# dongyunjinyu/YOLO-Lite

Hardware: NVIDIA B200
Metric: images_per_sec (higher is better)
Workload: dtype bf16

## Files before the change

### yolo-lite_b200/csrc/c3k2_fused.cu

```cuda
#include "common.cuh"

namespace yl {

struct C3k2TailParams {
    const __nv_bfloat16* t;
    long long t_cstride;
    int t_coff;
    __nv_bfloat16* y;
    long long y_cstride;
    int y_coff;
    const __nv_bfloat16 *wa, *wb, *w2;
    const float *ba, *bb, *b2;
    int wa_rows, wa_k, wb_k, w2_k;
    int N, H, W, C2, add;
    int tiles_w, tiles_h, total_tiles;
};

__device__ __forceinline__ void ldsm_x4(uint32_t addr, uint32_t& r0, uint32_t& r1, uint32_t& r2, uint32_t& r3) {
    asm volatile("ldmatrix.sync.aligned.m8n8.x4.shared.b16 {%0,%1,%2,%3}, [%4];"
                 : "=r"(r0), "=r"(r1), "=r"(r2), "=r"(r3)
                 : "r"(addr));
}
__device__ __forceinline__ void ldsm_x2(uint32_t addr, uint32_t& r0, uint32_t& r1) {
    asm volatile("ldmatrix.sync.aligned.m8n8.x2.shared.b16 {%0,%1}, [%2];" : "=r"(r0), "=r"(r1) : "r"(addr));
}
__device__ __forceinline__ void mma16816(float (&d)[4], const uint32_t (&a)[4], uint32_t b0, uint32_t b1) {
    asm volatile(
        "mma.sync.aligned.m16n8k16.row.col.f32.bf16.bf16.f32 {%0,%1,%2,%3}, {%4,%5,%6,%7}, {%8,%9}, {%0,%1,%2,%3};"
        : "+f"(d[0]), "+f"(d[1]), "+f"(d[2]), "+f"(d[3])
        : "r"(a[0]), "r"(a[1]), "r"(a[2]), "r"(a[3]), "r"(b0), "r"(b1));
}

__host__ __device__ constexpr int pitch16(int data_bytes) { return data_bytes + (((data_bytes / 16) & 1) ? 32 : 16); }

template <int C>
struct C3k2Smem {
    static constexpr int CH = C / 2;
    static constexpr int TH = (C == 16) ? 16 : 8, TW = 16;
    static constexpr int PH = TH + 4, PW = TW + 4;
    static constexpr int HH = TH + 2, HW = TW + 2;
    static constexpr int TS = pitch16(4 * C);
    static constexpr int HS = pitch16(2 * CH);
    static constexpr int YS = pitch16(2 * C);
    static constexpr int KA = 9 * C, KB = 9 * CH, K2 = 3 * C;
    static constexpr int WAS = pitch16(2 * KA), WBS = pitch16(2 * KB + 16), W2S = pitch16(2 * K2);
    static constexpr int NA = CH < 16 ? 8 : CH;
    static constexpr int HM = (HH * HW + 15) / 16;
    static constexpr int NBUF = C == 16 ? 2 : 1;
    static constexpr int T_BYTES = PH * PW * TS;
    static constexpr int off_t = 0;
    static constexpr int off_h = off_t + NBUF * T_BYTES;
    static constexpr int off_y2 = off_h + HM * 16 * HS;
    static constexpr int off_wa = off_y2 + TH * TW * YS;
    static constexpr int off_wb = off_wa + NA * WAS;
    static constexpr int off_w2 = off_wb + C * WBS;
    __host__ __device__ static constexpr int w2_bytes(int c2) { return c2 * W2S; }
    __host__ __device__ static constexpr int bias_floats(int c2) { return NA + C + c2; }
    __host__ __device__ static constexpr int total(int c2) { return off_w2 + w2_bytes(c2) + bias_floats(c2) * 4; }
};

__device__ __forceinline__ void stage_weights(uint8_t* dst, const __nv_bfloat16* src, int rows, int src_rows, int kbytes,
                                              int pitch) {
    const int units = pitch / 16;
    for (int i = threadIdx.x; i < rows * units; i += blockDim.x) {
        const int r = i / units, u = i - r * units;
        uint4 v = make_uint4(0u, 0u, 0u, 0u);
        if (r < src_rows && u * 16 < kbytes)
            v = __ldg(reinterpret_cast<const uint4*>(reinterpret_cast<const uint8_t*>(src) + (size_t)r * kbytes) + u);
        *reinterpret_cast<uint4*>(dst + (size_t)r * pitch + u * 16) = v;
    }
}

template <int C>
__global__ void __launch_bounds__(256, 2) c3k2_tail_kernel(const C3k2TailParams p) {
    using S = C3k2Smem<C>;
    constexpr int CH = S::CH, TH = S::TH, TW = S::TW, PW = S::PW, HW = S::HW, HH = S::HH;
    constexpr int TS = S::TS, HS = S::HS, YS = S::YS, WAS = S::WAS, WBS = S::WBS, W2S = S::W2S;
    extern __shared__ __align__(16) uint8_t smem[];
    griddep_launch_dependents();
    const int lane = threadIdx.x & 31, warp = threadIdx.x >> 5;
    const int g = lane >> 2, t = lane & 3;
    const int lrow = lane & 15, khalf = lane >> 4;
    const uint32_t sT = smem_u32(smem + S::off_t), sH = smem_u32(smem + S::off_h), sY2 = smem_u32(smem + S::off_y2);
    const uint32_t sWa = smem_u32(smem + S::off_wa), sWb = smem_u32(smem + S::off_wb), sW2 = smem_u32(smem + S::off_w2);
    float* sba = reinterpret_cast<float*>(smem + S::off_w2 + S::w2_bytes(p.C2));
    float* sbb = sba + S::NA;
    float* sb2 = sbb + C;

    stage_weights(smem + S::off_wa, p.wa, S::NA, p.wa_rows, p.wa_k * 2, WAS);
    stage_weights(smem + S::off_wb, p.wb, C, C, p.wb_k * 2, WBS);
    stage_weights(smem + S::off_w2, p.w2, p.C2, p.C2, p.w2_k * 2, W2S);
    for (int i = threadIdx.x; i < S::NA; i += blockDim.x) sba[i] = i < CH ? __ldg(p.ba + i) : 0.f;
    for (int i = threadIdx.x; i < C; i += blockDim.x) sbb[i] = __ldg(p.bb + i);
    for (int i = threadIdx.x; i < p.C2; i += blockDim.x) sb2[i] = __ldg(p.b2 + i);
    __syncthreads();

    constexpr int KT = 2 * C / 16, KY = C / 16, KC = KT + KY;
    const int NG = p.C2 / 32;
    const int grp = warp % NG, rblk = warp / NG;
    uint32_t bC[KC][4][2];
#pragma unroll
    for (int ks = 0; ks < KC; ++ks)
#pragma unroll
        for (int np = 0; np < 2; ++np)
            ldsm_x4(sW2 + (uint32_t)((grp * 32 + np * 16 + (lane >> 4) * 8 + (lane & 7)) * W2S + (ks * 16 + 8 * ((lane >> 3) & 1)) * 2),
                    bC[ks][2 * np][0], bC[ks][2 * np][1], bC[ks][2 * np + 1][0], bC[ks][2 * np + 1][1]);
    constexpr bool THIN = (C == 16);
    constexpr int KSB = (9 * CH + 15) / 16;
    uint32_t bA[THIN ? 9 : 1][2];
    if (THIN) {
#pragma unroll
        for (int tap = 0; tap < 9; ++tap)
            ldsm_x2(sWa + (uint32_t)((lane & 7) * WAS + (tap * C + 8 * ((lane >> 3) & 1)) * 2), bA[THIN ? tap : 0][0],
                    bA[THIN ? tap : 0][1]);
    }
    griddep_wait();

    constexpr int CHUNKS = 4 * C / 16;
    auto load_patch = [&](int tile, uint32_t dst) {
        const int w0 = (tile % p.tiles_w) * TW;
        const int h0 = ((tile / p.tiles_w) % p.tiles_h) * TH;
        const int n = tile / (p.tiles_w * p.tiles_h);
        const __nv_bfloat16* src0 = p.t + (long long)n * p.H * p.W * p.t_cstride + p.t_coff;
        for (int idx = threadIdx.x; idx < S::PH * PW * CHUNKS; idx += blockDim.x) {
            const int pix = idx / CHUNKS, ck = idx - pix * CHUNKS;
            const int pr = pix / PW, pc = pix - pr * PW;
            const int hi = h0 - 2 + pr, wi = w0 - 2 + pc;
            const bool ok = hi >= 0 && hi < p.H && wi >= 0 && wi < p.W;
            const int off = ok ? hi * p.W + wi : 0;
            asm volatile("cp.async.cg.shared.global [%0], [%1], 16, %2;" ::"r"(dst + (uint32_t)(pix * TS + ck * 16)),
                         "l"(src0 + (long long)off * p.t_cstride + ck * 8), "r"(ok ? 16 : 0)
                         : "memory");
        }
        asm volatile("cp.async.commit_group;" ::: "memory");
    };

    int buf = 0;
    if (S::NBUF == 2 && (int)blockIdx.x < p.total_tiles) load_patch(blockIdx.x, sT);
    for (int tile = blockIdx.x; tile < p.total_tiles; tile += gridDim.x) {
        const int w0 = (tile % p.tiles_w) * TW;
        const int h0 = ((tile / p.tiles_w) % p.tiles_h) * TH;
        const int n = tile / (p.tiles_w * p.tiles_h);
        const uint32_t sTc = sT + (uint32_t)(buf * S::T_BYTES);
        if (S::NBUF == 1) load_patch(tile, sTc);
        asm volatile("cp.async.wait_group 0;" ::: "memory");
        __syncthreads();
        if (S::NBUF == 2) {
            if (tile + (int)gridDim.x < p.total_tiles) load_patch(tile + gridDim.x, sT + (uint32_t)((buf ^ 1) * S::T_BYTES));
            buf ^= 1;
        }

        {
            constexpr int NT = (CH + 7) / 8;
            constexpr int KS_TAP = C / 16;
            for (int mt = warp; mt < S::HM; mt += 8) {
                int idx = mt * 16 + lrow;
                idx = idx < HH * HW ? idx : HH * HW - 1;
                const int hr = idx / HW, hc = idx - hr * HW;
                const uint32_t arow = sTc + (uint32_t)((hr * PW + hc) * TS + (C + 8 * khalf) * 2);
                float acc[NT][4];
#pragma unroll
                for (int nt = 0; nt < NT; ++nt) {
                    const float2 bb2 = *reinterpret_cast<const float2*>(sba + nt * 8 + 2 * t);
                    acc[nt][0] = bb2.x; acc[nt][1] = bb2.y; acc[nt][2] = bb2.x; acc[nt][3] = bb2.y;
                }
                if (THIN) {
                    uint32_t a9[9][4];
#pragma unroll
                    for (int tap = 0; tap < 9; ++tap)
                        ldsm_x4(arow + (uint32_t)(((tap / 3) * PW + tap % 3) * TS), a9[tap][0], a9[tap][1], a9[tap][2], a9[tap][3]);
#pragma unroll
                    for (int tap = 0; tap < 9; ++tap) mma16816(acc[0], a9[tap], bA[THIN ? tap : 0][0], bA[THIN ? tap : 0][1]);
                } else {
#pragma unroll
                    for (int tap = 0; tap < 9; ++tap) {
                        const int dr = tap / 3, dc = tap - 3 * dr;
                        uint32_t a[KS_TAP][4], b[KS_TAP][4];
#pragma unroll
                        for (int ks = 0; ks < KS_TAP; ++ks) {
                            ldsm_x4(arow + (uint32_t)((dr * PW + dc) * TS + ks * 32), a[ks][0], a[ks][1], a[ks][2], a[ks][3]);
                            ldsm_x4(sWa + (uint32_t)((((lane >> 4) * 8) + (lane & 7)) * WAS + (tap * C + ks * 16 + 8 * ((lane >> 3) & 1)) * 2),
                                    b[ks][0], b[ks][1], b[ks][2], b[ks][3]);
                        }
#pragma unroll
                        for (int ks = 0; ks < KS_TAP; ++ks) {
                            mma16816(acc[0], a[ks], b[ks][0], b[ks][1]);
                            mma16816(acc[NT - 1], a[ks], b[ks][2], b[ks][3]);
                        }
                    }
                }
#pragma unroll
                for (int half = 0; half < 2; ++half) {
                    const int e = mt * 16 + g + half * 8;
                    if (e >= HH * HW) continue;
                    const int er = e / HW, ec = e - er * HW;
                    const int hi = h0 - 1 + er, wi = w0 - 1 + ec;
                    const bool in = hi >= 0 && hi < p.H && wi >= 0 && wi < p.W;
#pragma unroll
                    for (int nt = 0; nt < NT; ++nt) {
                        const float v0 = in ? silu_fast(acc[nt][half * 2]) : 0.f;
                        const float v1 = in ? silu_fast(acc[nt][half * 2 + 1]) : 0.f;
                        asm volatile("st.shared.b32 [%0], %1;" ::"r"(sH + (uint32_t)(e * HS + (nt * 8 + 2 * t) * 2)),
                                     "r"(pack_bf16x2(v0, v1))
                                     : "memory");
                    }
                }
            }
        }
        __syncthreads();

        for (int r = warp; r < TH; r += 8) {
            constexpr int NT = C / 8;
            float acc[NT][4];
#pragma unroll
            for (int nt = 0; nt < NT; ++nt) {
                const float2 bb2 = *reinterpret_cast<const float2*>(sbb + nt * 8 + 2 * t);
                acc[nt][0] = bb2.x; acc[nt][1] = bb2.y; acc[nt][2] = bb2.x; acc[nt][3] = bb2.y;
            }
            const uint32_t hrow = sH + (uint32_t)((r * HW + lrow) * HS);
            if (CH == 8) {
                uint32_t a[KSB][4], b[KSB][4];
#pragma unroll
                for (int ks = 0; ks < KSB; ++ks) {
                    const int tap = min(2 * ks + khalf, 8);
                    const int dr = tap / 3, dc = tap - 3 * dr;
                    ldsm_x4(hrow + (uint32_t)((dr * HW + dc) * HS), a[ks][0], a[ks][1], a[ks][2], a[ks][3]);
                    ldsm_x4(sWb + (uint32_t)(((lane >> 4) * 8 + (lane & 7)) * WBS + (ks * 16 + 8 * ((lane >> 3) & 1)) * 2),
                            b[ks][0], b[ks][1], b[ks][2], b[ks][3]);
                }
#pragma unroll
                for (int ks = 0; ks < KSB; ++ks) {
                    mma16816(acc[0], a[ks], b[ks][0], b[ks][1]);
                    mma16816(acc[1], a[ks], b[ks][2], b[ks][3]);
                }
            } else {
                constexpr int KS_TAP = CH / 16;
#pragma unroll
                for (int k3 = 0; k3 < KSB; k3 += 3) {
                    uint32_t a[3][4], b[3][NT / 2][4];
#pragma unroll
                    for (int j = 0; j < 3; ++j) {
                        const int ks = k3 + j;
                        const int tap = ks / KS_TAP, kk = ks - tap * KS_TAP;
                        const int dr = tap / 3, dc = tap - 3 * dr;
                        ldsm_x4(hrow + (uint32_t)((dr * HW + dc) * HS + (kk * 16 + 8 * khalf) * 2), a[j][0], a[j][1], a[j][2], a[j][3]);
#pragma unroll
                        for (int np = 0; np < NT / 2; ++np)
                            ldsm_x4(sWb + (uint32_t)((np * 16 + (lane >> 4) * 8 + (lane & 7)) * WBS + (ks * 16 + 8 * ((lane >> 3) & 1)) * 2),
                                    b[j][np][0], b[j][np][1], b[j][np][2], b[j][np][3]);
                    }
#pragma unroll
                    for (int j = 0; j < 3; ++j)
#pragma unroll
                        for (int np = 0; np < NT / 2; ++np) {
                            mma16816(acc[2 * np], a[j], b[j][np][0], b[j][np][1]);
                            mma16816(acc[2 * np + 1], a[j], b[j][np][2], b[j][np][3]);
                        }
                }
            }
#pragma unroll
            for (int half = 0; half < 2; ++half) {
                const int col = g + half * 8;
                const uint32_t y1p = sTc + (uint32_t)(((r + 2) * PW + col + 2) * TS + C * 2);
                const uint32_t y2p = sY2 + (uint32_t)((r * TW + col) * YS);
#pragma unroll
                for (int nt = 0; nt < NT; ++nt) {
                    float v0 = silu_fast(acc[nt][half * 2]), v1 = silu_fast(acc[nt][half * 2 + 1]);
                    if (p.add) {
                        uint32_t rv;
                        asm volatile("ld.shared.b32 %0, [%1];" : "=r"(rv) : "r"(y1p + (uint32_t)((nt * 8 + 2 * t) * 2)));
                        v0 += bf16lo_f(rv);
                        v1 += bf16hi_f(rv);
                    }
                    asm volatile("st.shared.b32 [%0], %1;" ::"r"(y2p + (uint32_t)((nt * 8 + 2 * t) * 2)), "r"(pack_bf16x2(v0, v1))
                                 : "memory");
                }
            }
        }
        __syncthreads();

        {
            const int scol = g + 8 * (t >> 1);
            const int wi = w0 + scol;
            const int rpw = TH * NG / 8;
            for (int rr = 0; rr < rpw; ++rr) {
                const int r = rblk * rpw + rr;
                uint32_t a[KC][4];
                const uint32_t trow = sTc + (uint32_t)(((r + 2) * PW + lrow + 2) * TS + 8 * khalf * 2);
                const uint32_t yrow = sY2 + (uint32_t)((r * TW + lrow) * YS + 8 * khalf * 2);
#pragma unroll
                for (int ks = 0; ks < KT; ++ks) ldsm_x4(trow + ks * 32, a[ks][0], a[ks][1], a[ks][2], a[ks][3]);
#pragma unroll
                for (int ks = 0; ks < KY; ++ks) ldsm_x4(yrow + ks * 32, a[KT + ks][0], a[KT + ks][1], a[KT + ks][2], a[KT + ks][3]);
                float acc[4][4];
#pragma unroll
                for (int nt = 0; nt < 4; ++nt) {
                    const float2 bb2 = *reinterpret_cast<const float2*>(sb2 + grp * 32 + nt * 8 + 2 * t);
                    acc[nt][0] = bb2.x; acc[nt][1] = bb2.y; acc[nt][2] = bb2.x; acc[nt][3] = bb2.y;
                }
#pragma unroll
                for (int ks = 0; ks < KC; ++ks)
#pragma unroll
                    for (int nt = 0; nt < 4; ++nt) mma16816(acc[nt], a[ks], bC[ks][nt][0], bC[ks][nt][1]);
                const int hi = h0 + r;
                const bool st_ok = hi < p.H && wi < p.W;
                __nv_bfloat16* yp = p.y + (((long long)n * p.H + hi) * p.W + wi) * p.y_cstride + p.y_coff + grp * 32 + 8 * (t & 1);
#pragma unroll
                for (int np = 0; np < 2; ++np) {
                    uint32_t v0 = pack_bf16x2(silu_fast(acc[2 * np][0]), silu_fast(acc[2 * np][1]));
                    uint32_t v1 = pack_bf16x2(silu_fast(acc[2 * np + 1][0]), silu_fast(acc[2 * np + 1][1]));
                    uint32_t v2 = pack_bf16x2(silu_fast(acc[2 * np][2]), silu_fast(acc[2 * np][3]));
                    uint32_t v3 = pack_bf16x2(silu_fast(acc[2 * np + 1][2]), silu_fast(acc[2 * np + 1][3]));
                    {
                        const uint32_t s0 = (t & 1) ? v0 : v1, s1 = (t & 1) ? v2 : v3;
                        const uint32_t r0 = __shfl_xor_sync(0xffffffffu, s0, 1), r1 = __shfl_xor_sync(0xffffffffu, s1, 1);
                        if (t & 1) { v0 = r0; v2 = r1; } else { v1 = r0; v3 = r1; }
                    }
                    {
                        const uint32_t s0 = (t & 2) ? v0 : v2, s1 = (t & 2) ? v1 : v3;
                        const uint32_t r0 = __shfl_xor_sync(0xffffffffu, s0, 2), r1 = __shfl_xor_sync(0xffffffffu, s1, 2);
                        if (t & 2) { v0 = r0; v1 = r1; } else { v2 = r0; v3 = r1; }
                    }
                    if (st_ok) *reinterpret_cast<uint4*>(yp + np * 16) = make_uint4(v0, v1, v2, v3);
                }
            }
        }
        __syncthreads();
    }
}

static int g_c3k2_sms = 148, g_c3k2_max_smem = 0;

template <int C>
static int launch_c3k2_tail(C3k2TailParams p, cudaStream_t s) {
    using S = C3k2Smem<C>;
    p.tiles_w = ceil_div(p.W, S::TW);
    p.tiles_h = ceil_div(p.H, S::TH);
    p.total_tiles = p.tiles_w * p.tiles_h * p.N;
    const size_t smem = (size_t)S::total(p.C2);
    YL_CHECK((int)smem <= g_c3k2_max_smem, YL_ERR_UNSUPPORTED, "c3k2 tail needs %zu B of shared memory (device allows %d)", smem,
             g_c3k2_max_smem);
    int per_sm = (int)((size_t)220 * 1024 / (smem + 1024));
    per_sm = per_sm < 1 ? 1 : (per_sm > 2 ? 2 : per_sm);
    int grid = g_c3k2_sms * per_sm;
    if (grid > p.total_tiles) grid = p.total_tiles;
    YL_CUDA(launch_kernel(c3k2_tail_kernel<C>, dim3(grid), dim3(256), smem, s, p));
    YL_LAUNCH_OK("c3k2_tail_kernel");
    return YL_OK;
}

int init_c3k2() {
    int dev = 0;
    YL_CUDA(cudaGetDevice(&dev));
    YL_CUDA(cudaDeviceGetAttribute(&g_c3k2_sms, cudaDevAttrMultiProcessorCount, dev));
    YL_CUDA(cudaDeviceGetAttribute(&g_c3k2_max_smem, cudaDevAttrMaxSharedMemoryPerBlockOptin, dev));
    YL_CUDA(cudaFuncSetAttribute(c3k2_tail_kernel<16>, cudaFuncAttributeMaxDynamicSharedMemorySize, g_c3k2_max_smem));
    YL_CUDA(cudaFuncSetAttribute(c3k2_tail_kernel<32>, cudaFuncAttributeMaxDynamicSharedMemorySize, g_c3k2_max_smem));
    return YL_OK;
}

}

namespace yl {
bool c3k2_tc_supported(int c, int c2);
int launch_c3k2_tc(const yl_tensor* t, const yl_tensor* y, const void* wa, const float* ba, int wa_ci_pad, const void* wb,
                   const float* bb, int wb_ci_pad, const void* w2, const float* b2, int w2_ci_pad, int shortcut,
                   cudaStream_t stream);
}

extern "C" int yl_c3k2_tail_tc(const yl_tensor* t, const yl_tensor* y, const void* wa, const float* ba, int wa_co_pad,
                               int wa_ci_pad, const void* wb, const float* bb, int wb_ci_pad, const void* w2,
                               const float* b2, int w2_ci_pad, int shortcut, void* stream) {
    YL_CHECK(t && y && t->data && y->data && wa && wb && w2 && ba && bb && b2, YL_ERR_ARG, "null pointer");
    YL_CHECK(t->dtype == YL_BF16 && y->dtype == YL_BF16, YL_ERR_ARG, "c3k2 tail tensors must be bf16");
    YL_CHECK(t->n == y->n && t->h == y->h && t->w == y->w && t->c % 32 == 0, YL_ERR_ARG, "c3k2 tail shape mismatch");
    YL_CHECK(t->coff % 8 == 0 && t->cstride % 8 == 0 && y->coff % 8 == 0 && y->cstride % 8 == 0, YL_ERR_ARG,
             "c3k2 tail needs 8-channel alignment");
    const int c = t->c / 2;
    YL_CHECK(wa_co_pad >= c / 2 && wa_ci_pad == c && wb_ci_pad == (c / 2 + 7) / 8 * 8 && w2_ci_pad == 3 * c, YL_ERR_ARG,
             "packed weight layouts do not match the block");
    return yl::launch_c3k2_tc(t, y, wa, ba, wa_ci_pad, wb, bb, wb_ci_pad, w2, b2, w2_ci_pad, shortcut, (cudaStream_t)stream);
}

extern "C" int yl_c3k2_tail_supported(int c, int c2) {
    return (c == 16 || c == 32) && (c2 == 32 || c2 == 64 || c2 == 128 || c2 == 256);
}

extern "C" int yl_c3k2_tail(const yl_tensor* t, const yl_tensor* y, const void* wa, const float* ba, int wa_co_pad,
                            int wa_ci_pad, const void* wb, const float* bb, int wb_ci_pad, const void* w2, const float* b2,
                            int w2_ci_pad, int shortcut, void* stream) {
    YL_CHECK(t && y && t->data && y->data && wa && wb && w2 && ba && bb && b2, YL_ERR_ARG, "null pointer");
    YL_CHECK(t->dtype == YL_BF16 && y->dtype == YL_BF16, YL_ERR_ARG, "c3k2 tail tensors must be bf16");
    YL_CHECK(t->n == y->n && t->h == y->h && t->w == y->w, YL_ERR_ARG, "c3k2 tail shape mismatch");
    YL_CHECK(t->c % 32 == 0 && yl_c3k2_tail_supported(t->c / 2, y->c), YL_ERR_UNSUPPORTED,
             "c3k2 tail is built for c in {16, 32} and c2 in {32, 64, 128, 256} (got c = %d, c2 = %d)", t->c / 2, y->c);
    YL_CHECK(t->coff % 8 == 0 && t->cstride % 8 == 0 && y->coff % 8 == 0 && y->cstride % 8 == 0, YL_ERR_ARG,
             "c3k2 tail needs 8-channel alignment");
    YL_CHECK(((uintptr_t)t->data | (uintptr_t)y->data | (uintptr_t)wa | (uintptr_t)wb | (uintptr_t)w2) % 16 == 0, YL_ERR_ARG,
             "pointers must be 16-byte aligned");
    const int c = t->c / 2;
    YL_CHECK(wa_ci_pad == c && wb_ci_pad == (c / 2 + 7) / 8 * 8 && w2_ci_pad == 3 * c, YL_ERR_ARG,
             "packed weight layouts do not match the block (ci_pad %d / %d / %d for c = %d)", wa_ci_pad, wb_ci_pad,
             w2_ci_pad, c);
    YL_CHECK((long long)t->h * t->w < (1ll << 31), YL_ERR_ARG, "image too large");
    if (yl::c3k2_tc_supported(c, y->c))
        return yl::launch_c3k2_tc(t, y, wa, ba, wa_ci_pad, wb, bb, wb_ci_pad, w2, b2, w2_ci_pad, shortcut, (cudaStream_t)stream);
    yl::C3k2TailParams p;
    p.t = reinterpret_cast<const __nv_bfloat16*>(t->data);
    p.t_cstride = t->cstride;
    p.t_coff = t->coff;
    p.y = reinterpret_cast<__nv_bfloat16*>(y->data);
    p.y_cstride = y->cstride;
    p.y_coff = y->coff;
    p.wa = reinterpret_cast<const __nv_bfloat16*>(wa);
    p.wb = reinterpret_cast<const __nv_bfloat16*>(wb);
    p.w2 = reinterpret_cast<const __nv_bfloat16*>(w2);
    p.ba = ba;
    p.bb = bb;
    p.b2 = b2;
    p.wa_rows = wa_co_pad;
    p.wa_k = 9 * wa_ci_pad;
    p.wb_k = 9 * wb_ci_pad;
    p.w2_k = w2_ci_pad;
    p.N = t->n;
    p.H = t->h;
    p.W = t->w;
    p.C2 = y->c;
    p.add = shortcut;
    cudaStream_t s = (cudaStream_t)stream;
    return c == 16 ? yl::launch_c3k2_tail<16>(p, s) : yl::launch_c3k2_tail<32>(p, s);
}
```

### yolo-lite_b200/csrc/stem_fused.cu

```cuda
#include <cuda_fp16.h>

#include "common.cuh"

namespace yl {

struct StemFusedParams {
    const void* x;
    int N, CI, H, W;
    const __nv_bfloat16* w0;
    int ci_pad0;
    const float* b0;
    const __nv_bfloat16* w1;
    const float* b1;
    __nv_bfloat16* y;
    long long y_cstride;
    int y_coff;
    int H0, W0, H1, W1;
    int act0, act1;
    int tiles_w, tiles_h, total_tiles;
};

__device__ __forceinline__ void sf_ldsm_x4(uint32_t addr, uint32_t& r0, uint32_t& r1, uint32_t& r2, uint32_t& r3) {
    asm volatile("ldmatrix.sync.aligned.m8n8.x4.shared.b16 {%0,%1,%2,%3}, [%4];"
                 : "=r"(r0), "=r"(r1), "=r"(r2), "=r"(r3)
                 : "r"(addr));
}
__device__ __forceinline__ void sf_mma(float (&d)[4], const uint32_t (&a)[4], uint32_t b0, uint32_t b1) {
    asm volatile(
        "mma.sync.aligned.m16n8k16.row.col.f32.bf16.bf16.f32 {%0,%1,%2,%3}, {%4,%5,%6,%7}, {%8,%9}, {%0,%1,%2,%3};"
        : "+f"(d[0]), "+f"(d[1]), "+f"(d[2]), "+f"(d[3])
        : "r"(a[0]), "r"(a[1]), "r"(a[2]), "r"(a[3]), "r"(b0), "r"(b1));
}

template <typename T> struct SfQuad;
template <> struct SfQuad<float> {
    using raw = float4;
    static __device__ __forceinline__ raw zero() { return make_float4(0.f, 0.f, 0.f, 0.f); }
    static __device__ __forceinline__ raw load(const float* p) { return __ldg(reinterpret_cast<const float4*>(p)); }
    static __device__ __forceinline__ float4 widen(raw v) { return v; }
    static __device__ __forceinline__ float one(const float* p) { return __ldg(p); }
};
template <> struct SfQuad<__half> {
    using raw = uint2;
    static __device__ __forceinline__ raw zero() { return make_uint2(0u, 0u); }
    static __device__ __forceinline__ raw load(const __half* p) { return __ldg(reinterpret_cast<const uint2*>(p)); }
    static __device__ __forceinline__ float4 widen(raw v) {
        const float2 a = __half22float2(*reinterpret_cast<const __half2*>(&v.x));
        const float2 b = __half22float2(*reinterpret_cast<const __half2*>(&v.y));
        return make_float4(a.x, a.y, b.x, b.y);
    }
    static __device__ __forceinline__ float one(const __half* p) { return __half2float(*p); }
};
template <> struct SfQuad<uint8_t> {
    using raw = uint32_t;
    static __device__ __forceinline__ raw zero() { return 0u; }
    static __device__ __forceinline__ raw load(const uint8_t* p) { return __ldg(reinterpret_cast<const uint32_t*>(p)); }
    static __device__ __forceinline__ float4 widen(raw v) {
        return make_float4(__fdiv_rn((float)(v & 0xffu), 255.f), __fdiv_rn((float)((v >> 8) & 0xffu), 255.f),
                           __fdiv_rn((float)((v >> 16) & 0xffu), 255.f), __fdiv_rn((float)(v >> 24), 255.f));
    }
    static __device__ __forceinline__ float one(const uint8_t* p) { return __fdiv_rn((float)__ldg(p), 255.f); }
};

constexpr int SF_TH = 8, SF_TW = 16;
constexpr int SF_R0 = 2 * SF_TH + 1, SF_C0 = 2 * SF_TW + 1;
constexpr int SF_RI = 2 * SF_R0 + 1;
constexpr int SF_CI = 72;
constexpr int SF_M0 = (SF_R0 * SF_C0 + 15) / 16;
constexpr int SF_EC = (SF_C0 + 1) / 2;
constexpr int SF_P0 = 48;
constexpr int SF_W1S = 9 * 16 * 2 + 16;
constexpr int SF_OFF_IN = 0;
constexpr int SF_OFF_L0 = SF_OFF_IN + SF_RI * SF_CI * 8;
constexpr int SF_OFF_W1 = SF_OFF_L0 + 2 * SF_R0 * SF_EC * SF_P0;
constexpr int SF_OFF_B = SF_OFF_W1 + 32 * SF_W1S;
constexpr int SF_OFF_TAB = SF_OFF_B + 48 * 4;
constexpr int SF_SMEM = SF_OFF_TAB + SF_M0 * 16 * 8;

template <typename TIn>
__global__ void __launch_bounds__(256, 2) stem_fused_kernel(const StemFusedParams p) {
    using Q = SfQuad<TIn>;
    const TIn* px_in = reinterpret_cast<const TIn*>(p.x);
    extern __shared__ __align__(16) uint8_t sf_smem[];
    griddep_launch_dependents();
    const int lane = threadIdx.x & 31, warp = threadIdx.x >> 5;
    const int g = lane >> 2, t = lane & 3;
    uint2* s_in = reinterpret_cast<uint2*>(sf_smem + SF_OFF_IN);
    const uint32_t sL0 = smem_u32(sf_smem + SF_OFF_L0), sW1 = smem_u32(sf_smem + SF_OFF_W1);
    float* sb0 = reinterpret_cast<float*>(sf_smem + SF_OFF_B);
    float* sb1 = sb0 + 16;

    for (int i = threadIdx.x; i < 32 * (SF_W1S / 16); i += blockDim.x) {
        const int r = i / (SF_W1S / 16), u = i - r * (SF_W1S / 16);
        uint4 v = make_uint4(0u, 0u, 0u, 0u);
        if (u < 18) v = __ldg(reinterpret_cast<const uint4*>(p.w1 + (size_t)r * 144) + u);
        *reinterpret_cast<uint4*>(sf_smem + SF_OFF_W1 + r * SF_W1S + u * 16) = v;
    }
    if (threadIdx.x < 16) sb0[threadIdx.x] = __ldg(p.b0 + threadIdx.x);
    if (threadIdx.x < 32) sb1[threadIdx.x] = __ldg(p.b1 + threadIdx.x);
    uint32_t bw0[3][2][2];
#pragma unroll
    for (int nt = 0; nt < 2; ++nt) {
        const __nv_bfloat16* wrow = p.w0 + (size_t)(nt * 8 + g) * 9 * p.ci_pad0;
#pragma unroll
        for (int ks = 0; ks < 3; ++ks)
#pragma unroll
            for (int hh = 0; hh < 2; ++hh) {
                uint32_t v = 0;
#pragma unroll
                for (int e = 0; e < 2; ++e) {
                    const int k = 16 * ks + 2 * t + e + hh * 8;
                    const int tap = k >> 2, ci = k & 3;
                    uint32_t bits = 0;
                    if (tap < 9 && ci < p.CI) bits = (uint32_t)__bfloat16_as_ushort(wrow[tap * p.ci_pad0 + ci]);
                    v |= bits << (16 * e);
                }
                bw0[ks][nt][hh] = v;
            }
    }
    int woff[3][2];
#pragma unroll
    for (int ks = 0; ks < 3; ++ks)
#pragma unroll
        for (int hh = 0; hh < 2; ++hh) {
            const int k = 16 * ks + 2 * t + hh * 8;
            const int tap = k >> 2, r = tap / 3, s2 = tap - 3 * r;
            woff[ks][hh] = tap < 9 ? ((r * SF_CI + s2) * 2 + ((k >> 1) & 1)) : 0;
        }
    uint2* s_tab = reinterpret_cast<uint2*>(sf_smem + SF_OFF_TAB);
    for (int i = threadIdx.x; i < SF_M0 * 16; i += blockDim.x) {
        const bool valid = i < SF_R0 * SF_C0;
        const int idx = valid ? i : SF_R0 * SF_C0 - 1;
        const int er = idx / SF_C0, ec = idx - er * SF_C0;
        const uint32_t aoff = (uint32_t)(((2 * er) * SF_CI + 2 * ec + 1) * 2);
        const uint32_t doff = (uint32_t)((((ec & 1) * SF_R0 + er) * SF_EC + (ec >> 1)) * SF_P0);
        s_tab[i] = make_uint2(aoff | ((uint32_t)(valid ? er : 255) << 16) | ((uint32_t)ec << 24), doff);
    }
    griddep_wait();

    const long long plane = (long long)p.H * p.W;
    const bool vec_ok = (p.W & 3) == 0 && ((reinterpret_cast<uintptr_t>(p.x) & (4 * sizeof(TIn) - 1)) == 0);
    constexpr int QUADS = SF_CI / 4;
    constexpr int ITEMS = SF_RI * QUADS;
    constexpr int ROUNDS = (ITEMS + 255) / 256;
    typename Q::raw pf[ROUNDS][3];

    auto patch_issue = [&](int tile) {
        const int ow0 = (tile % p.tiles_w) * SF_TW;
        const int oh0 = ((tile / p.tiles_w) % p.tiles_h) * SF_TH;
        const int n = tile / (p.tiles_w * p.tiles_h);
        const int ir0 = 4 * oh0 - 3, ic0 = 4 * ow0 - 4;
        const TIn* xn = px_in + (long long)n * p.CI * plane;
#pragma unroll
        for (int j = 0; j < ROUNDS; ++j) {
            const int item = threadIdx.x + j * 256;
            const int pr = item / QUADS, q = item - pr * QUADS;
            const int hi = ir0 + pr, wi0 = ic0 + 4 * q;
            const bool ok = item < ITEMS && hi >= 0 && hi < p.H && wi0 >= 0 && wi0 < p.W;
            const TIn* src0 = xn + (long long)(ok ? hi : 0) * p.W + (ok ? wi0 : 0);
#pragma unroll
            for (int ci = 0; ci < 3; ++ci) {
                pf[j][ci] = Q::zero();
                if (ok && ci < p.CI) pf[j][ci] = Q::load(src0 + ci * plane);
            }
        }
    };
    auto patch_store = [&]() {
#pragma unroll
        for (int j = 0; j < ROUNDS; ++j) {
            const int item = threadIdx.x + j * 256;
            if (item >= ITEMS) continue;
            const int pr = item / QUADS, q = item - pr * QUADS;
            uint4* dst = reinterpret_cast<uint4*>(s_in + pr * SF_CI + 4 * q);
            const float4 c0 = Q::widen(pf[j][0]), c1 = Q::widen(pf[j][1]), c2 = Q::widen(pf[j][2]);
            dst[0] = make_uint4(pack_bf16x2(c0.x, c1.x), pack_bf16x2(c2.x, 0.f), pack_bf16x2(c0.y, c1.y), pack_bf16x2(c2.y, 0.f));
            dst[1] = make_uint4(pack_bf16x2(c0.z, c1.z), pack_bf16x2(c2.z, 0.f), pack_bf16x2(c0.w, c1.w), pack_bf16x2(c2.w, 0.f));
        }
    };
    auto patch_slow = [&](int tile) {
        const int ow0 = (tile % p.tiles_w) * SF_TW;
        const int oh0 = ((tile / p.tiles_w) % p.tiles_h) * SF_TH;
        const int n = tile / (p.tiles_w * p.tiles_h);
        const int ir0 = 4 * oh0 - 3, ic0 = 4 * ow0 - 4;
        const TIn* xn = px_in + (long long)n * p.CI * plane;
        for (int item = threadIdx.x; item < ITEMS; item += blockDim.x) {
            const int pr = item / QUADS, q = item - pr * QUADS;
            const int hi = ir0 + pr, wi0 = ic0 + 4 * q;
            float v[3][4];
#pragma unroll
            for (int ci = 0; ci < 3; ++ci)
#pragma unroll
                for (int e = 0; e < 4; ++e) {
                    v[ci][e] = 0.f;
                    if (ci < p.CI && hi >= 0 && hi < p.H && wi0 + e >= 0 && wi0 + e < p.W)
                        v[ci][e] = Q::one(xn + ci * plane + (long long)hi * p.W + wi0 + e);
                }
            uint4* dst = reinterpret_cast<uint4*>(s_in + pr * SF_CI + 4 * q);
            dst[0] = make_uint4(pack_bf16x2(v[0][0], v[1][0]), pack_bf16x2(v[2][0], 0.f), pack_bf16x2(v[0][1], v[1][1]),
                                pack_bf16x2(v[2][1], 0.f));
            dst[1] = make_uint4(pack_bf16x2(v[0][2], v[1][2]), pack_bf16x2(v[2][2], 0.f), pack_bf16x2(v[0][3], v[1][3]),
                                pack_bf16x2(v[2][3], 0.f));
        }
    };

    if ((int)blockIdx.x < p.total_tiles) {
        if (vec_ok) {
            patch_issue(blockIdx.x);
            patch_store();
        } else {
            patch_slow(blockIdx.x);
        }
    }
    __syncthreads();
    for (int tile = blockIdx.x; tile < p.total_tiles; tile += gridDim.x) {
        const int ow0 = (tile % p.tiles_w) * SF_TW;
        const int oh0 = ((tile / p.tiles_w) % p.tiles_h) * SF_TH;
        const int n = tile / (p.tiles_w * p.tiles_h);
        const int next = tile + (int)gridDim.x;

        {
            const uint32_t* pw = reinterpret_cast<const uint32_t*>(s_in);
            const int er_lo = oh0 == 0 ? 1 : 0, er_hi = min(SF_R0, p.H0 - (2 * oh0 - 1));
            const int ec_lo = ow0 == 0 ? 1 : 0, ec_hi = min(SF_C0, p.W0 - (2 * ow0 - 1));
            for (int mt = warp; mt < SF_M0; mt += 8) {
                uint32_t a[3][4];
                uint2 te[2];
#pragma unroll
                for (int half = 0; half < 2; ++half) {
                    te[half] = s_tab[mt * 16 + g + half * 8];
                    const uint32_t* px = pw + (te[half].x & 0xffffu);
#pragma unroll
                    for (int ks = 0; ks < 3; ++ks) {
                        a[ks][half] = px[woff[ks][0]];
                        a[ks][2 + half] = px[woff[ks][1]];
                    }
                }
                float acc[2][4];
#pragma unroll
                for (int nt = 0; nt < 2; ++nt) {
                    const float2 bb = *reinterpret_cast<const float2*>(sb0 + nt * 8 + 2 * t);
                    acc[nt][0] = bb.x; acc[nt][1] = bb.y; acc[nt][2] = bb.x; acc[nt][3] = bb.y;
#pragma unroll
                    for (int ks = 0; ks < 3; ++ks) sf_mma(acc[nt], a[ks], bw0[ks][nt][0], bw0[ks][nt][1]);
                }
#pragma unroll
                for (int half = 0; half < 2; ++half) {
                    const int er = (int)((te[half].x >> 16) & 0xffu), ec = (int)(te[half].x >> 24);
                    if (er == 255) continue;
                    const bool in = er >= er_lo && er < er_hi && ec >= ec_lo && ec < ec_hi;
                    const uint32_t dst = sL0 + te[half].y + (uint32_t)(4 * t);
#pragma unroll
                    for (int nt = 0; nt < 2; ++nt) {
                        float v0 = acc[nt][half * 2], v1 = acc[nt][half * 2 + 1];
                        if (p.act0) {
                            v0 = silu_fast(v0);
                            v1 = silu_fast(v1);
                        }
                        asm volatile("st.shared.b32 [%0], %1;" ::"r"(dst + (uint32_t)(nt * 16)), "r"(in ? pack_bf16x2(v0, v1) : 0u)
                                     : "memory");
                    }
                }
            }
        }
        __syncthreads();
        if (vec_ok && next < p.total_tiles) patch_issue(next);

        {
            const int r = warp;
            const int lrow = lane & 15, khalf = lane >> 4;
            float acc[4][4];
#pragma unroll
            for (int nt = 0; nt < 4; ++nt) {
                const float2 bb = *reinterpret_cast<const float2*>(sb1 + nt * 8 + 2 * t);
                acc[nt][0] = bb.x; acc[nt][1] = bb.y; acc[nt][2] = bb.x; acc[nt][3] = bb.y;
            }
            const uint32_t brow = sW1 + (uint32_t)(((lane >> 4) * 8 + (lane & 7)) * SF_W1S + 8 * ((lane >> 3) & 1) * 2);
#pragma unroll
            for (int t3 = 0; t3 < 9; t3 += 3) {
                uint32_t a[3][4], b[3][2][4];
#pragma unroll
                for (int j = 0; j < 3; ++j) {
                    const int tap = t3 + j, dr = tap / 3, dc = tap - 3 * dr;
                    const uint32_t arow = sL0 + (uint32_t)((((dc & 1) * SF_R0 + 2 * r + dr) * SF_EC + lrow + (dc >> 1)) * SF_P0 +
                                                           khalf * 16);
                    sf_ldsm_x4(arow, a[j][0], a[j][1], a[j][2], a[j][3]);
#pragma unroll
                    for (int np = 0; np < 2; ++np)
                        sf_ldsm_x4(brow + (uint32_t)(np * 16 * SF_W1S + tap * 32), b[j][np][0], b[j][np][1], b[j][np][2],
                                   b[j][np][3]);
                }
#pragma unroll
                for (int j = 0; j < 3; ++j)
#pragma unroll
                    for (int np = 0; np < 2; ++np) {
                        sf_mma(acc[2 * np], a[j], b[j][np][0], b[j][np][1]);
                        sf_mma(acc[2 * np + 1], a[j], b[j][np][2], b[j][np][3]);
                    }
            }
            const int oh = oh0 + r, ow = ow0 + g + 8 * (t >> 1);
            const bool st_ok = oh < p.H1 && ow < p.W1;
            __nv_bfloat16* yp = p.y + (((long long)n * p.H1 + oh) * p.W1 + ow) * p.y_cstride + p.y_coff + 8 * (t & 1);
#pragma unroll
            for (int np = 0; np < 2; ++np) {
                float e[2][4];
#pragma unroll
                for (int q = 0; q < 2; ++q)
#pragma unroll
                    for (int i = 0; i < 4; ++i) e[q][i] = p.act1 ? silu_fast(acc[2 * np + q][i]) : acc[2 * np + q][i];
                uint32_t v0 = pack_bf16x2(e[0][0], e[0][1]);
                uint32_t v1 = pack_bf16x2(e[1][0], e[1][1]);
                uint32_t v2 = pack_bf16x2(e[0][2], e[0][3]);
                uint32_t v3 = pack_bf16x2(e[1][2], e[1][3]);
                {
                    const uint32_t s0 = (t & 1) ? v0 : v1, s1 = (t & 1) ? v2 : v3;
                    const uint32_t r0 = __shfl_xor_sync(0xffffffffu, s0, 1), r1 = __shfl_xor_sync(0xffffffffu, s1, 1);
                    if (t & 1) { v0 = r0; v2 = r1; } else { v1 = r0; v3 = r1; }
                }
                {
                    const uint32_t s0 = (t & 2) ? v0 : v2, s1 = (t & 2) ? v1 : v3;
                    const uint32_t r0 = __shfl_xor_sync(0xffffffffu, s0, 2), r1 = __shfl_xor_sync(0xffffffffu, s1, 2);
                    if (t & 2) { v0 = r0; v1 = r1; } else { v2 = r0; v3 = r1; }
                }
                if (st_ok) *reinterpret_cast<uint4*>(yp + np * 16) = make_uint4(v0, v1, v2, v3);
            }
        }
        if (next < p.total_tiles) {
            if (vec_ok) patch_store();
            else patch_slow(next);
        }
        __syncthreads();
    }
}

static int g_sf_sms = 148;

int init_stem_fused() {
    int dev = 0;
    YL_CUDA(cudaGetDevice(&dev));
    YL_CUDA(cudaDeviceGetAttribute(&g_sf_sms, cudaDevAttrMultiProcessorCount, dev));
    YL_CUDA(cudaFuncSetAttribute(stem_fused_kernel<float>, cudaFuncAttributeMaxDynamicSharedMemorySize, SF_SMEM));
    YL_CUDA(cudaFuncSetAttribute(stem_fused_kernel<__half>, cudaFuncAttributeMaxDynamicSharedMemorySize, SF_SMEM));
    YL_CUDA(cudaFuncSetAttribute(stem_fused_kernel<uint8_t>, cudaFuncAttributeMaxDynamicSharedMemorySize, SF_SMEM));
    return YL_OK;
}

}

extern "C" int yl_stem_fused_supported(int ci, int c0, int c1) { return ci >= 1 && ci <= 3 && c0 == 16 && c1 == 32; }

extern "C" int yl_stem_fused(const void* x_nchw, int x_dtype, int n, int ci, int h, int w, const void* w0, int ci_pad0,
                             const float* b0, int act0, const void* w1, int ci_pad1, const float* b1, int act1,
                             const yl_tensor* y, void* stream) {
    YL_CHECK(x_nchw && w0 && b0 && w1 && b1 && y && y->data, YL_ERR_ARG, "null pointer");
    YL_CHECK(x_dtype == YL_F32 || x_dtype == YL_F16 || x_dtype == YL_U8, YL_ERR_ARG,
             "fused stem reads fp32, fp16 or uint8 images (got dtype %d)", x_dtype);
    YL_CHECK(y->dtype == YL_BF16, YL_ERR_ARG, "stem output must be bf16");
    YL_CHECK(yl_stem_fused_supported(ci, 16, y->c) && ci_pad1 == 16, YL_ERR_UNSUPPORTED,
             "fused stem is built for <= 3 input channels, 16 -> 32 (got ci = %d, c1 = %d, ci_pad1 = %d)", ci, y->c, ci_pad1);
    const int H0 = (h + 2 - 3) / 2 + 1, W0 = (w + 2 - 3) / 2 + 1;
    const int H1 = (H0 + 2 - 3) / 2 + 1, W1 = (W0 + 2 - 3) / 2 + 1;
    YL_CHECK(y->n == n && y->h == H1 && y->w == W1, YL_ERR_ARG, "fused stem output shape mismatch: got (%d,%d,%d) expected (%d,%d,%d)",
             y->n, y->h, y->w, n, H1, W1);
    YL_CHECK(y->coff % 8 == 0 && y->cstride % 8 == 0 && ((uintptr_t)y->data | (uintptr_t)w1) % 16 == 0, YL_ERR_ARG,
             "fused stem needs 8-channel / 16-byte alignment");
    YL_CHECK((long long)ci * h * w < (1ll << 31), YL_ERR_ARG, "image too large");
    yl::StemFusedParams p;
    p.x = x_nchw;
    p.N = n;
    p.CI = ci;
    p.H = h;
    p.W = w;
    p.w0 = reinterpret_cast<const __nv_bfloat16*>(w0);
    p.ci_pad0 = ci_pad0;
    p.b0 = b0;
    p.w1 = reinterpret_cast<const __nv_bfloat16*>(w1);
    p.b1 = b1;
    p.y = reinterpret_cast<__nv_bfloat16*>(y->data);
    p.y_cstride = y->cstride;
    p.y_coff = y->coff;
    p.H0 = H0;
    p.W0 = W0;
    p.H1 = H1;
    p.W1 = W1;
    p.act0 = act0;
    p.act1 = act1;
    p.tiles_w = yl::ceil_div(W1, yl::SF_TW);
    p.tiles_h = yl::ceil_div(H1, yl::SF_TH);
    p.total_tiles = p.tiles_w * p.tiles_h * n;
    const int sms = yl::g_sf_sms;
    int per_sm = (int)((size_t)220 * 1024 / (yl::SF_SMEM + 1024));
    per_sm = per_sm < 1 ? 1 : (per_sm > 2 ? 2 : per_sm);
    int grid = sms * per_sm;
    if (grid > p.total_tiles) grid = p.total_tiles;
    if (x_dtype == YL_F32)
        YL_CUDA(yl::launch_kernel(yl::stem_fused_kernel<float>, dim3(grid), dim3(256), (size_t)yl::SF_SMEM, (cudaStream_t)stream, p));
    else if (x_dtype == YL_F16)
        YL_CUDA(yl::launch_kernel(yl::stem_fused_kernel<__half>, dim3(grid), dim3(256), (size_t)yl::SF_SMEM, (cudaStream_t)stream, p));
    else
        YL_CUDA(yl::launch_kernel(yl::stem_fused_kernel<uint8_t>, dim3(grid), dim3(256), (size_t)yl::SF_SMEM, (cudaStream_t)stream, p));
    YL_LAUNCH_OK("stem_fused_kernel");
    return YL_OK;
}
```

Baseline: 41070.

## Keep conv weights in registers and prefetch stem input via cp.async

```diff
diff --git a/yolo-lite_b200/csrc/c3k2_fused.cu b/yolo-lite_b200/csrc/c3k2_fused.cu
--- a/yolo-lite_b200/csrc/c3k2_fused.cu
+++ b/yolo-lite_b200/csrc/c3k2_fused.cu
@@ -108,11 +108,16 @@
     constexpr bool THIN = (C == 16);
     constexpr int KSB = (9 * CH + 15) / 16;
     uint32_t bA[THIN ? 9 : 1][2];
+    uint32_t bB[THIN ? KSB : 1][4];
     if (THIN) {
 #pragma unroll
         for (int tap = 0; tap < 9; ++tap)
             ldsm_x2(sWa + (uint32_t)((lane & 7) * WAS + (tap * C + 8 * ((lane >> 3) & 1)) * 2), bA[THIN ? tap : 0][0],
                     bA[THIN ? tap : 0][1]);
+#pragma unroll
+        for (int ks = 0; ks < (THIN ? KSB : 1); ++ks)
+            ldsm_x4(sWb + (uint32_t)(((lane >> 4) * 8 + (lane & 7)) * WBS + (ks * 16 + 8 * ((lane >> 3) & 1)) * 2), bB[ks][0],
+                    bB[ks][1], bB[ks][2], bB[ks][3]);
     }
     griddep_wait();
 
@@ -219,19 +224,19 @@
             }
             const uint32_t hrow = sH + (uint32_t)((r * HW + lrow) * HS);
             if (CH == 8) {
-                uint32_t a[KSB][4], b[KSB][4];
+                uint32_t a[KSB][4];
 #pragma unroll
                 for (int ks = 0; ks < KSB; ++ks) {
                     const int tap = min(2 * ks + khalf, 8);
                     const int dr = tap / 3, dc = tap - 3 * dr;
                     ldsm_x4(hrow + (uint32_t)((dr * HW + dc) * HS), a[ks][0], a[ks][1], a[ks][2], a[ks][3]);
-                    ldsm_x4(sWb + (uint32_t)(((lane >> 4) * 8 + (lane & 7)) * WBS + (ks * 16 + 8 * ((lane >> 3) & 1)) * 2),
-                            b[ks][0], b[ks][1], b[ks][2], b[ks][3]);
                 }
 #pragma unroll
                 for (int ks = 0; ks < KSB; ++ks) {
-                    mma16816(acc[0], a[ks], b[ks][0], b[ks][1]);
-                    mma16816(acc[1], a[ks], b[ks][2], b[ks][3]);
+                    const int kb = THIN ? ks : 0;
+                    const bool pad = ks == KSB - 1;
+                    mma16816(acc[0], a[ks], bB[kb][0], pad ? 0u : bB[kb][1]);
+                    mma16816(acc[1], a[ks], bB[kb][2], pad ? 0u : bB[kb][3]);
                 }
             } else {
                 constexpr int KS_TAP = CH / 16;
diff --git a/yolo-lite_b200/csrc/stem_fused.cu b/yolo-lite_b200/csrc/stem_fused.cu
--- a/yolo-lite_b200/csrc/stem_fused.cu
+++ b/yolo-lite_b200/csrc/stem_fused.cu
@@ -35,15 +35,11 @@
 template <typename T> struct SfQuad;
 template <> struct SfQuad<float> {
     using raw = float4;
-    static __device__ __forceinline__ raw zero() { return make_float4(0.f, 0.f, 0.f, 0.f); }
-    static __device__ __forceinline__ raw load(const float* p) { return __ldg(reinterpret_cast<const float4*>(p)); }
     static __device__ __forceinline__ float4 widen(raw v) { return v; }
     static __device__ __forceinline__ float one(const float* p) { return __ldg(p); }
 };
 template <> struct SfQuad<__half> {
     using raw = uint2;
-    static __device__ __forceinline__ raw zero() { return make_uint2(0u, 0u); }
-    static __device__ __forceinline__ raw load(const __half* p) { return __ldg(reinterpret_cast<const uint2*>(p)); }
     static __device__ __forceinline__ float4 widen(raw v) {
         const float2 a = __half22float2(*reinterpret_cast<const __half2*>(&v.x));
         const float2 b = __half22float2(*reinterpret_cast<const __half2*>(&v.y));
@@ -53,8 +49,6 @@
 };
 template <> struct SfQuad<uint8_t> {
     using raw = uint32_t;
-    static __device__ __forceinline__ raw zero() { return 0u; }
-    static __device__ __forceinline__ raw load(const uint8_t* p) { return __ldg(reinterpret_cast<const uint32_t*>(p)); }
     static __device__ __forceinline__ float4 widen(raw v) {
         return make_float4(__fdiv_rn((float)(v & 0xffu), 255.f), __fdiv_rn((float)((v >> 8) & 0xffu), 255.f),
                            __fdiv_rn((float)((v >> 16) & 0xffu), 255.f), __fdiv_rn((float)(v >> 24), 255.f));
@@ -69,13 +63,22 @@
 constexpr int SF_M0 = (SF_R0 * SF_C0 + 15) / 16;
 constexpr int SF_EC = (SF_C0 + 1) / 2;
 constexpr int SF_P0 = 48;
-constexpr int SF_W1S = 9 * 16 * 2 + 16;
 constexpr int SF_OFF_IN = 0;
 constexpr int SF_OFF_L0 = SF_OFF_IN + SF_RI * SF_CI * 8;
-constexpr int SF_OFF_W1 = SF_OFF_L0 + 2 * SF_R0 * SF_EC * SF_P0;
-constexpr int SF_OFF_B = SF_OFF_W1 + 32 * SF_W1S;
+constexpr int SF_OFF_B = SF_OFF_L0 + 2 * SF_R0 * SF_EC * SF_P0;
 constexpr int SF_OFF_TAB = SF_OFF_B + 48 * 4;
-constexpr int SF_SMEM = SF_OFF_TAB + SF_M0 * 16 * 8;
+constexpr int SF_QUADS = SF_RI * (SF_CI / 4);
+constexpr int SF_OFF_RAW = SF_OFF_TAB + SF_M0 * 16 * 8;
+constexpr int SF_SMEM = SF_OFF_RAW + 3 * SF_QUADS * 16;
+
+template <int bytes>
+__device__ __forceinline__ void sf_cp_async(uint32_t dst, const void* src, bool ok) {
+    if constexpr (bytes == 16)
+        asm volatile("cp.async.cg.shared.global [%0], [%1], 16, %2;" ::"r"(dst), "l"(src), "r"(ok ? 16 : 0) : "memory");
+    else
+        asm volatile("cp.async.ca.shared.global [%0], [%1], %2, %3;" ::"r"(dst), "l"(src), "n"(bytes), "r"(ok ? bytes : 0)
+                     : "memory");
+}
 
 template <typename TIn>
 __global__ void __launch_bounds__(256, 2) stem_fused_kernel(const StemFusedParams p) {
@@ -86,16 +89,10 @@
     const int lane = threadIdx.x & 31, warp = threadIdx.x >> 5;
     const int g = lane >> 2, t = lane & 3;
     uint2* s_in = reinterpret_cast<uint2*>(sf_smem + SF_OFF_IN);
-    const uint32_t sL0 = smem_u32(sf_smem + SF_OFF_L0), sW1 = smem_u32(sf_smem + SF_OFF_W1);
+    const uint32_t sL0 = smem_u32(sf_smem + SF_OFF_L0);
     float* sb0 = reinterpret_cast<float*>(sf_smem + SF_OFF_B);
     float* sb1 = sb0 + 16;
 
-    for (int i = threadIdx.x; i < 32 * (SF_W1S / 16); i += blockDim.x) {
-        const int r = i / (SF_W1S / 16), u = i - r * (SF_W1S / 16);
-        uint4 v = make_uint4(0u, 0u, 0u, 0u);
-        if (u < 18) v = __ldg(reinterpret_cast<const uint4*>(p.w1 + (size_t)r * 144) + u);
-        *reinterpret_cast<uint4*>(sf_smem + SF_OFF_W1 + r * SF_W1S + u * 16) = v;
-    }
     if (threadIdx.x < 16) sb0[threadIdx.x] = __ldg(p.b0 + threadIdx.x);
     if (threadIdx.x < 32) sb1[threadIdx.x] = __ldg(p.b1 + threadIdx.x);
     uint32_t bw0[3][2][2];
@@ -117,6 +114,17 @@
                 }
                 bw0[ks][nt][hh] = v;
             }
+    }
+    const int nh = warp & 1, rq = warp >> 1;
+    uint32_t bw1[9][2][2];
+#pragma unroll
+    for (int nt = 0; nt < 2; ++nt) {
+        const __nv_bfloat16* wrow = p.w1 + (size_t)(16 * nh + 8 * nt + g) * 144 + 2 * t;
+#pragma unroll
+        for (int tap = 0; tap < 9; ++tap)
+#pragma unroll
+            for (int hh = 0; hh < 2; ++hh)
+                bw1[tap][nt][hh] = __ldg(reinterpret_cast<const uint32_t*>(wrow + tap * 16 + hh * 8));
     }
     int woff[3][2];
 #pragma unroll
@@ -141,9 +149,10 @@
     const long long plane = (long long)p.H * p.W;
     const bool vec_ok = (p.W & 3) == 0 && ((reinterpret_cast<uintptr_t>(p.x) & (4 * sizeof(TIn) - 1)) == 0);
     constexpr int QUADS = SF_CI / 4;
-    constexpr int ITEMS = SF_RI * QUADS;
+    constexpr int ITEMS = SF_QUADS;
     constexpr int ROUNDS = (ITEMS + 255) / 256;
-    typename Q::raw pf[ROUNDS][3];
+    constexpr int QB = (int)sizeof(typename Q::raw);
+    const uint32_t sRaw = smem_u32(sf_smem + SF_OFF_RAW);
 
     auto patch_issue = [&](int tile) {
         const int ow0 = (tile % p.tiles_w) * SF_TW;
@@ -154,25 +163,28 @@
 #pragma unroll
         for (int j = 0; j < ROUNDS; ++j) {
             const int item = threadIdx.x + j * 256;
+            if (item >= ITEMS) continue;
             const int pr = item / QUADS, q = item - pr * QUADS;
             const int hi = ir0 + pr, wi0 = ic0 + 4 * q;
-            const bool ok = item < ITEMS && hi >= 0 && hi < p.H && wi0 >= 0 && wi0 < p.W;
+            const bool ok = hi >= 0 && hi < p.H && wi0 >= 0 && wi0 < p.W;
             const TIn* src0 = xn + (long long)(ok ? hi : 0) * p.W + (ok ? wi0 : 0);
 #pragma unroll
-            for (int ci = 0; ci < 3; ++ci) {
-                pf[j][ci] = Q::zero();
-                if (ok && ci < p.CI) pf[j][ci] = Q::load(src0 + ci * plane);
-            }
-        }
+            for (int ci = 0; ci < 3; ++ci)
+                sf_cp_async<QB>(sRaw + (uint32_t)((ci * ITEMS + item) * QB), src0 + (ci < p.CI ? ci * plane : 0),
+                                ok && ci < p.CI);
+        }
+        asm volatile("cp.async.commit_group;" ::: "memory");
     };
     auto patch_store = [&]() {
+        asm volatile("cp.async.wait_group 0;" ::: "memory");
+        const typename Q::raw* raw = reinterpret_cast<const typename Q::raw*>(sf_smem + SF_OFF_RAW);
 #pragma unroll
         for (int j = 0; j < ROUNDS; ++j) {
             const int item = threadIdx.x + j * 256;
             if (item >= ITEMS) continue;
             const int pr = item / QUADS, q = item - pr * QUADS;
             uint4* dst = reinterpret_cast<uint4*>(s_in + pr * SF_CI + 4 * q);
-            const float4 c0 = Q::widen(pf[j][0]), c1 = Q::widen(pf[j][1]), c2 = Q::widen(pf[j][2]);
+            const float4 c0 = Q::widen(raw[item]), c1 = Q::widen(raw[ITEMS + item]), c2 = Q::widen(raw[2 * ITEMS + item]);
             dst[0] = make_uint4(pack_bf16x2(c0.x, c1.x), pack_bf16x2(c2.x, 0.f), pack_bf16x2(c0.y, c1.y), pack_bf16x2(c2.y, 0.f));
             dst[1] = make_uint4(pack_bf16x2(c0.z, c1.z), pack_bf16x2(c2.z, 0.f), pack_bf16x2(c0.w, c1.w), pack_bf16x2(c2.w, 0.f));
         }
@@ -217,6 +229,7 @@
         const int oh0 = ((tile / p.tiles_w) % p.tiles_h) * SF_TH;
         const int n = tile / (p.tiles_w * p.tiles_h);
         const int next = tile + (int)gridDim.x;
+        if (vec_ok && next < p.total_tiles) patch_issue(next);
 
         {
             const uint32_t* pw = reinterpret_cast<const uint32_t*>(s_in);
@@ -263,50 +276,40 @@
             }
         }
         __syncthreads();
-        if (vec_ok && next < p.total_tiles) patch_issue(next);
-
-        {
-            const int r = warp;
-            const int lrow = lane & 15, khalf = lane >> 4;
-            float acc[4][4];
-#pragma unroll
-            for (int nt = 0; nt < 4; ++nt) {
-                const float2 bb = *reinterpret_cast<const float2*>(sb1 + nt * 8 + 2 * t);
+
+        const int lrow = lane & 15, khalf = lane >> 4;
+#pragma unroll 1
+        for (int r = rq; r < SF_TH; r += 4) {
+            float acc[2][4];
+#pragma unroll
+            for (int nt = 0; nt < 2; ++nt) {
+                const float2 bb = *reinterpret_cast<const float2*>(sb1 + (2 * nh + nt) * 8 + 2 * t);
                 acc[nt][0] = bb.x; acc[nt][1] = bb.y; acc[nt][2] = bb.x; acc[nt][3] = bb.y;
             }
-            const uint32_t brow = sW1 + (uint32_t)(((lane >> 4) * 8 + (lane & 7)) * SF_W1S + 8 * ((lane >> 3) & 1) * 2);
 #pragma unroll
             for (int t3 = 0; t3 < 9; t3 += 3) {
-                uint32_t a[3][4], b[3][2][4];
+                uint32_t a[3][4];
 #pragma unroll
                 for (int j = 0; j < 3; ++j) {
                     const int tap = t3 + j, dr = tap / 3, dc = tap - 3 * dr;
                     const uint32_t arow = sL0 + (uint32_t)((((dc & 1) * SF_R0 + 2 * r + dr) * SF_EC + lrow + (dc >> 1)) * SF_P0 +
                                                            khalf * 16);
                     sf_ldsm_x4(arow, a[j][0], a[j][1], a[j][2], a[j][3]);
-#pragma unroll
-                    for (int np = 0; np < 2; ++np)
-                        sf_ldsm_x4(brow + (uint32_t)(np * 16 * SF_W1S + tap * 32), b[j][np][0], b[j][np][1], b[j][np][2],
-                                   b[j][np][3]);
                 }
 #pragma unroll
                 for (int j = 0; j < 3; ++j)
 #pragma unroll
-                    for (int np = 0; np < 2; ++np) {
-                        sf_mma(acc[2 * np], a[j], b[j][np][0], b[j][np][1]);
-                        sf_mma(acc[2 * np + 1], a[j], b[j][np][2], b[j][np][3]);
-                    }
+                    for (int nt = 0; nt < 2; ++nt) sf_mma(acc[nt], a[j], bw1[t3 + j][nt][0], bw1[t3 + j][nt][1]);
             }
             const int oh = oh0 + r, ow = ow0 + g + 8 * (t >> 1);
             const bool st_ok = oh < p.H1 && ow < p.W1;
-            __nv_bfloat16* yp = p.y + (((long long)n * p.H1 + oh) * p.W1 + ow) * p.y_cstride + p.y_coff + 8 * (t & 1);
-#pragma unroll
-            for (int np = 0; np < 2; ++np) {
+            __nv_bfloat16* yp = p.y + (((long long)n * p.H1 + oh) * p.W1 + ow) * p.y_cstride + p.y_coff + 16 * nh + 8 * (t & 1);
+            {
                 float e[2][4];
 #pragma unroll
                 for (int q = 0; q < 2; ++q)
 #pragma unroll
-                    for (int i = 0; i < 4; ++i) e[q][i] = p.act1 ? silu_fast(acc[2 * np + q][i]) : acc[2 * np + q][i];
+                    for (int i = 0; i < 4; ++i) e[q][i] = p.act1 ? silu_fast(acc[q][i]) : acc[q][i];
                 uint32_t v0 = pack_bf16x2(e[0][0], e[0][1]);
                 uint32_t v1 = pack_bf16x2(e[1][0], e[1][1]);
                 uint32_t v2 = pack_bf16x2(e[0][2], e[0][3]);
@@ -321,7 +324,7 @@
                     const uint32_t r0 = __shfl_xor_sync(0xffffffffu, s0, 2), r1 = __shfl_xor_sync(0xffffffffu, s1, 2);
                     if (t & 2) { v0 = r0; v1 = r1; } else { v2 = r0; v3 = r1; }
                 }
-                if (st_ok) *reinterpret_cast<uint4*>(yp + np * 16) = make_uint4(v0, v1, v2, v3);
+                if (st_ok) *reinterpret_cast<uint4*>(yp) = make_uint4(v0, v1, v2, v3);
             }
         }
         if (next < p.total_tiles) {
```

After: 41460 (median of 6 runs). No clear change (+1.0%).
